# sajadn/Exemplar-VAE

Hardware: AMD Instinct MI355X
Metric: training images/sec (higher is better)
Workload: dtype f32

## Files before the change

### exemplar-vae_amd/csrc/evae_prior.hip

```cpp
#include <algorithm>
#include <type_traits>
#include "evae_tile.h"
#include "evae_prior_gemm.h"

namespace evae {

constexpr long long kMaskAll = EVAE_PRIOR_MASK_ALL;

__device__ __forceinline__ float setup_sigma(float* __restrict__ inv_sigma, float* __restrict__ red,
                                             const float* __restrict__ log_var, int zdim, int zpad) {
  float part = 0.f;
  for (int k = threadIdx.x; k < zpad; k += NT) {
    float lv = k < zdim ? log_var[k] : 0.f;
    inv_sigma[k] = k < zdim ? expf(-0.5f * lv) : 0.f;
    if (k < zdim) part += lv + kLog2Pi;
  }
  part = wave_sum(part);
  if ((threadIdx.x & 63) == 0) red[threadIdx.x >> 6] = part;
  __syncthreads();
  float tot = red[0] + red[1] + red[2] + red[3];
  return -0.5f * tot;
}

template <int KC>
// ... 1719 lines not shown
  return check_launch("prior_bwd_finish_kernel");
}

extern "C" int evae_prior_train_step(const float* z, int B, const float* centres, int C, int zdim, const float* log_var,
                                     const int64_t* z_idx, const int64_t* c_idx, float c_total, const float* beta_dev,
                                     float beta_host, float* logp, float* token, float* cRE, float* cKL, float* neg_cKL,
                                     float* dz, float* dcentres, float* dlogvar, void* state, void* ws, size_t ws_bytes,
                                     int phase, evae_stream_t stream_) {
  return prior_train_step_core(z, B, centres, C, zdim, log_var, z_idx, c_idx, c_total, beta_dev, beta_host, logp, token, cRE, cKL, neg_cKL,
                               dz, dcentres, dlogvar, state, ws, ws_bytes, phase, stream_, nullptr, nullptr, nullptr, 0, nullptr);
}

extern "C" int evae_prior_train_step_rows(const float* z, int B, const float* centres, int n_rows, const int64_t* rows_inv,
                                          const int64_t* rows_rep, const float* rows_mult, int C, int zdim, const float* log_var,
                                          const int64_t* z_idx, const int64_t* c_idx, float c_total, const float* beta_dev,
                                          float beta_host, float* logp, float* token, float* cRE, float* cKL, float* neg_cKL,
                                          float* dz, float* dcentres, float* dc_draws, float* dlogvar, void* state, void* ws,
                                          size_t ws_bytes, evae_stream_t stream_) {
  EVAE_REQUIRE(rows_inv && rows_rep && rows_mult && dc_draws && n_rows >= 1, "prior_train_step_rows: null row tables");
  EVAE_REQUIRE((((uintptr_t)dc_draws | (uintptr_t)dcentres) & 15) == 0, "prior_train_step_rows: gradient buffers must be 16-byte aligned");
  return prior_train_step_core(z, B, centres, C, zdim, log_var, z_idx, c_idx, c_total, beta_dev, beta_host, logp, token, cRE, cKL, neg_cKL,
                               dz, dcentres, dlogvar, state, ws, ws_bytes, 0, stream_, rows_inv, rows_rep, rows_mult, n_rows, dc_draws);
}
```

### exemplar-vae_amd/evae/_lib.py

```python
import ctypes as C
import os

_HERE = os.path.dirname(os.path.abspath(__file__))
LIB_PATH = os.environ.get("EVAE_LIB_PATH") or os.path.join(os.path.dirname(_HERE), "csrc", "libevae_hip.so")

_p = C.c_void_p
_i = C.c_int
_f = C.c_float
_d = C.c_double
_z = C.c_size_t
_l = C.c_int64
_u = C.c_uint
_q = C.c_uint64


class ConvDesc(C.Structure):
    _fields_ = [(n, C.c_int) for n in ("N", "C", "H", "W", "Co", "KH", "KW", "stride", "pad")]


class WtJob(C.Structure):
    _fields_ = [("w1", C.c_void_p), ("w2", C.c_void_p), ("dst", C.c_void_p), ("N", C.c_int), ("K", C.c_int), ("ldt", C.c_int)]


class CtlJob(C.Structure):
# ... 20 lines not shown
class AdamTensor(C.Structure):
    _fields_ = [("param", _p), ("grad", _p), ("exp_avg", _p), ("exp_avg_sq", _p), ("numel", _l)]


SIGNATURES = {
    "evae_version": (_i, []),
    "evae_last_error": (C.c_char_p, []),
    "evae_ctl_upload": (_i, [_p, _p, _p, _z, _p, _p, _p, _p]),
    "evae_host_dedup": (_i, [_p, _i, C.c_int64, _i, _p, _p, _p, _p]),
    "evae_prior_set_norm_limit": (_i, [_f]),
    "evae_prior_lse_fwd_workspace_bytes": (_z, [_i, _i, _i]),
    "evae_prior_lse_fwd": (_i, [_p, _i, _p, _i, _i, _p, _p, _p, _p, _p, _p, _p, _p, _z, _p]),
    "evae_prior_merge": (_i, [_p, _p, _p, _i, _i, _f, _p, _p, _p]),
    "evae_prior_lse_fwd_splits": (_i, [_p, _i, _p, _i, _i, _p, _p, _p, _p, _z, C.POINTER(C.c_int), C.POINTER(C.c_int), _p]),
    "evae_prior_elbo_fwd": (_i, [_p, _p, _p, _i, _i, _i, _f, _p, _p, _p, _f, _p, _p, _p, _p, _p, _p]),
    "evae_prior_elbo_fwd_coef": (_i, [_p, _p, _p, _i, _i, _i, _f, _p, _p, _p, _f, _p, _p, _p, _p, _p, _p, _p, _p, _p]),
    "evae_prior_merge_coef": (_i, [_p, _p, _p, _i, _i, _i, _f, _p, _f, _p, _p, _p, _p, _p, _p]),
    "evae_elbo_assemble": (_i, [_p, _p, _p, _p, _f, _i, _p, _p, _p, _p]),
    "evae_prior_train_applies": (_i, [_i, _i, _i]),
    "evae_prior_train_gave_up": (_i, [_p, _p]),
    "evae_prior_train_workspace_bytes": (_z, [_i, _i, _i]),
    "evae_prior_train_step": (_i, [_p, _i, _p, _i, _i, _p, _p, _p, _f, _p, _f, _p, _p, _p, _p, _p, _p, _p, _p, _p, _p, _z, _i, _p]),
    "evae_prior_train_step_rows": (_i, [_p, _i, _p, _i, _p, _p, _p, _i, _i, _p, _p, _p, _f, _p, _f, _p, _p, _p, _p, _p, _p, _p, _p, _p, _p, _p, _z, _p]),
    "evae_prior_lse_bwd_workspace_bytes": (_z, [_i, _i, _i]),
    "evae_prior_lse_bwd": (_i, [_p, _i, _p, _i, _i, _p, _p, _p, _p, _p, _p, _p, _p, _p, _z, _p]),
    "evae_prior_lse_bwd_phased": (_i, [_p, _i, _p, _i, _i, _p, _p, _p, _p, _p, _p, _p, _p, _p, _z, _i, _p]),
    "evae_mixture_lse_fwd_workspace_bytes": (_z, [_i, _i, _i]),
    "evae_mixture_lse_fwd": (_i, [_p, _i, _p, _p, _i, _i, _f, _p, _p, _p, _p, _z, _p]),
    "evae_mixture_lse_bwd_workspace_bytes": (_z, [_i, _i, _i]),
    "evae_mixture_lse_bwd": (_i, [_p, _i, _p, _p, _i, _i, _p, _p, _p, _p, _p, _p, _z, _p]),
    "evae_pseudo_inputs_fwd": (_i, [_p, _i, _i, _p, _p]),
    "evae_pseudo_inputs_bwd": (_i, [_p, _p, _i, _i, _p, _p]),
    "evae_pairdist_topk_workspace_bytes": (_z, [_i, _i, _i, _i]),
    "evae_pairdist_topk": (_i, [_p, _i, _p, _i, _i, _i, _u, _l, _p, _p, _p, _z, _p]),
    "evae_pairwise_distance": (_i, [_p, _i, _p, _i, _i, _p, _p]),
    "evae_topk_merge": (_i, [_p, _p, _i, _i, _i, _p, _p, _p]),
    "evae_select_exemplars": (_i, [_p, _i, _p, _i, _p, _p, _p, _p]),
    "evae_dense_fwd_workspace_bytes": (_z, [_i, _i, _i, _i]),
    "evae_gated_dense_fwd": (_i, [_p, _p, _i, _i, _i, _p, _p, _p, _p, _i, _p, _p, _p, _p, _z, _p]),
    "evae_linear_fwd": (_i, [_p, _p, _i, _i, _i, _p, _p, _i, _i, _f, _f, _p, _p, _p, _z, _p]),
    "evae_heads_reparam_fwd_workspace_bytes": (_z, [_i, _i, _i]),
    "evae_heads_reparam_fwd": (_i, [_p, _i, _i, _i, _p, _p, _p, _p, _i, _f, _f, _p, _p, _p, _p, _p, _p, _p, _z, _p]),
    "evae_heads_reparam_fwd_bcast_applies": (_i, [_i, _i, _i, _i]),
    "evae_heads_reparam_fwd_bcast": (_i, [_p, _i, _i, _i, _p, _p, _p, _p, _i, _f, _f, _p, _p, _p, _p, _p, _p, _p, _p, _i, _p]),
    "evae_heads_std_applies": (_i, [_i, _i, _i, _i]),
    "evae_heads_reparam_std_fwd": (_i, [_p, _i, _i, _i, _p, _p, _p, _p, _i, _f, _f, _p, _p, _p, _p, _p, _p, _p, _p]),
# ... 12 lines not shown
    "evae_dense_bwd_weight_phased": (_i, [_p, _i, _i, _i, _p, _p, _i, _i, _p, _p, _i, _p, _z, _i, _p]),
    "evae_dense_u8_supported": (_i, [_i, C.c_longlong]),
    "evae_dense_u8_block_rows": (_i, [_i, _i, _i]),
    "evae_dense_u8_prepared_bytes": (_z, [_i, _i]),
    "evae_dense_u8_prepare": (_i, [_p, _p, _i, _i, _p, _z, _p]),
    "evae_gated_dense_fwd_u8": (_i, [_p, _p, _i, _i, C.c_longlong, _f, _p, _p, _p, _i, _p, _p, _p]),
    "evae_dense_bwd_weight_u8_workspace_bytes": (_z, [_i, _i, _i]),
    "evae_dense_bwd_weight_u8": (_i, [_p, _i, _i, C.c_longlong, _p, _p, _i, C.c_longlong, _f, _p, _p, _p, _z, _p]),
    "evae_dense_bwd_weight_u8_phased": (_i, [_p, _i, _i, C.c_longlong, _p, _p, _i, C.c_longlong, _f, _p, _p, _p, _z, _i, _p]),
    "evae_dense_bwd_weight_u8_images": (_i, [_i, _i, _i, C.POINTER(C.c_size_t), C.POINTER(C.c_int)]),
    "evae_broadcast_scalar": (_i, [_p, _p, _i, _p]),
    "evae_sum_small": (_i, [_p, _i, _p, _p]),
    "evae_thin_configure": (_i, [_i]),
    "evae_p6_nks": (_i, [_i]),
    "evae_p6_nks_rows": (_i, [_i]),
    "evae_p6_image_bytes": (_z, [_i, _i]),
    "evae_gemm_p6_applies": (_i, [_i, _i, _i]),
    "evae_p6_pack_rows": (_i, [_p, _p, _i, _i, C.c_longlong, _i, _p, _z, _p]),
    "evae_p6_pack_cols": (_i, [_p, _p, _i, _i, C.c_longlong, _i, _i, _p, _z, _p]),
    "evae_p6_fill_row": (_i, [_p, _i, _i, _f, _i, _i, _p]),
    "evae_gated_dense_fwd_timg": (_i, [_p, _p, _i, _i, _i, _p, _p, _p, _p, _i, _p, _p, _p, _p, _i, _i, _i, _p, _z, _p]),
    "evae_gated_dense_fwd_u8_timg": (_i, [_p, _p, _i, _i, C.c_longlong, _f, _p, _p, _p, _i, _p, _p, _p, _i, _i, _i, _p]),
    "evae_dense_bwd_data_timg": (_i, [_p, _p, _p, _p, _i, _i, _i, _i, _p, _p, _p, _p, _i, _p, _p, _i, _i, _i, _p, _z, _p]),
    "evae_gated_dense_fwd_p6t": (_i, [_p, _i, _i, _i, _p, _p, _p, _i, _p, _p, _p]),
    "evae_dense_bwd_data_p6t": (_i, [_p, _i, _i, _i, _p, _i, _p, _p, _p, _p, _i, _p, _i, _i, _p]),
    "evae_dense_bwd_weight_p6_workspace_bytes": (_z, [_i, _i, _i]),
    "evae_dense_bwd_weight_p6": (_i, [_p, _p, _i, _i, _i, _p, _p, _p, _z, _p]),
    "evae_dense_bwd_data_img": (_i, [_p, _p, _p, _p, _i, _i, _i, _i, _p, _p, _p, _i, _i, _p, _p, _z, _p]),
    "evae_dense_bwd_weight_group": (_i, [_p, _i, _p]),
    "evae_dense_bwd_weight_finish_group": (_i, [_p, _i, _p]),
    "evae_gated_dense_bwd_input": (_i, [_p, _p, _p, _i, _i, _p, _p, _i, _p]),
    "evae_gated_dense_bwd_input_ld": (_i, [_p, _i, _p, _p, _i, _i, _p, _p, _i, _p]),
    "evae_gather_rows": (_i, [_p, _p, _p, _i, _i, _p, _p]),
    "evae_gated_dense_bwd": (_i, [_p, _i, _p, _p, _i, _i, _p, _p, _i, _p, _i, _p, _i, _p, _z, _p]),
    "evae_act_bwd": (_i, [_p, _p, _z, _i, _f, _f, _p, _p]),
    "evae_conv2d_workspace_bytes": (_z, [_p, _i, _i]),
    "evae_conv2d_fwd": (_i, [_p, _p, _p, _p, _p, _p, _i, _f, _f, _p, _p, _p, _p, _z, _p]),
    "evae_conv2d_bwd_data": (_i, [_p, _p, _p, _p, _p, _p, _p, _z, _p]),
    "evae_conv2d_bwd_weight": (_i, [_p, _p, _p, _p, _p, _p, _p, _z, _p]),
    "evae_conv2d_cl_supported": (_i, [_p, _i, _i]),
    "evae_conv2d_cl_dy_stride": (_i, [_i]),
    "evae_conv2d_cl_workspace_bytes": (_z, [_p, _i, _i]),
    "evae_conv2d_cl_fwd": (_i, [_p, _p, _p, _p, _p, _p, _i, _f, _f, _p, _p, _p, _p, _z, _p]),
    "evae_conv2d_cl_bwd_data": (_i, [_p, _p, _p, _p, _p, _p, _z, _p]),
    "evae_conv2d_cl_bwd_weight": (_i, [_p, _p, _p, _i, _p, _p, _p, _z, _p]),
    "evae_gemm_x6_configure": (_i, [_i, _i]),
# ... 123 lines not shown
```

### exemplar-vae_amd/evae/fused_vae.py

```python
import ctypes as C
import os

import torch
import torch.distributed as dist

from . import _lib, handoff, ops, shard

ACT_NONE, ACT_SIGMOID, ACT_HARDTANH = ops.ACT_NONE, ops.ACT_SIGMOID, ops.ACT_HARDTANH

_STAGE_GEN = {}
_XT_GEN = {}
_ZEROED = {}
def node_merge(Cl, B):
    e = os.environ.get("EVAE_NODE_MERGE")
    if e is not None:
        return int(e)
    return 15 if Cl + B <= 8192 else 11


ONE_STREAM = [os.environ.get("EVAE_ONE_STREAM", "0") == "1"]
_APPROX_ROWS = {}

SCHED = int(os.environ.get("EVAE_SCHED", "0"))
FINISH_GROUP_HEAD = os.environ.get("EVAE_FINISH_GROUP_HEAD", "0") == "1"
FINISH_GROUP = os.environ.get("EVAE_FINISH_GROUP", "0") == "1"
HEADW_EARLY = int(os.environ.get("EVAE_HEADW_EARLY", "0"))
ELBO_SPLIT = os.environ.get("EVAE_ELBO_SPLIT", "0") != "0"
PRIOR_TRAIN = os.environ.get("EVAE_PRIOR_TRAIN", "1") != "0"
GROUP_LEAVES = os.environ.get("EVAE_GROUP_LEAVES", "1") != "0"
IMG_DGRAD = os.environ.get("EVAE_IMG_DGRAD", "1") != "0" or bool(SCHED & 4)
THIN_ROWS = 1024
P6 = os.environ.get("EVAE_P6", "1") != "0"
_P6_READY = {}
_ONES = {}

PARAM_ORDER = [
    "prior_log_variance",
    "p_x_mean.linear.weight", "p_x_mean.linear.bias",
    "q_z_layers.0.h.weight", "q_z_layers.0.h.bias", "q_z_layers.0.g.weight", "q_z_layers.0.g.bias",
    "q_z_layers.1.h.weight", "q_z_layers.1.h.bias", "q_z_layers.1.g.weight", "q_z_layers.1.g.bias",
    "q_z_mean.weight", "q_z_mean.bias",
    "q_z_logvar.linear.weight", "q_z_logvar.linear.bias",
    "p_x_layers.0.h.weight", "p_x_layers.0.h.bias", "p_x_layers.0.g.weight", "p_x_layers.0.g.bias",
    "p_x_layers.1.h.weight", "p_x_layers.1.h.bias", "p_x_layers.1.g.weight", "p_x_layers.1.g.bias",
]




def _vp(v):
    if v is None:
        return None
    return C.c_void_p(v if isinstance(v, int) else v.data_ptr())


# ... 268 lines not shown
                           lambda: _lib.check(lib.evae_gated_dense_fwd_p6t(_vp(t_h1), nks_m, Cl, H, _vp(w2_img), _vp(b2h), _vp(b2g), H,
                                                                           _vp(A2), _vp(s2), k.st), "gated_fwd_p6t"),
                           executed=6 * fl2, pipe="bf16-mfma")
            else:
                k.gated_fwd(A1, None, Cl, H, H, w2h, b2h, w2g, b2g, H, A2, None, s2)
            k.linear_fwd(A2, Cl, H, H, wm, bm, Z, ACT_NONE, 0.0, 0.0, mean_all, None)
        if approx:
            approx_cache.index_copy_(0, sel_rows, centres)
        main.wait_event(z_ready)
        centres_p = centres
        if dd is not None and not prior_train:
            centres_p = torch.empty((Cp, Z), **f32)
            _lib.check(lib.evae_gather_rows(_vp(centres), _vp(dd[1]), None, Cp, Z, _vp(centres_p), k.st), "gather_rows(centres)")
        zi = None if no_mask else ops._i64(x_idx)
        ci = None if no_mask else (ci_sel if approx else ops._i64(dd[0] if dd is not None else ex_idx))
        logp = torch.empty(B, **f32); lse = torch.empty((2, B), **f32)
        z_all, zi_all = z, zi
        prior_done = None
        if prior_train:
            dmean_all = torch.empty((Mp, Z), **f32)
            packed = torch.empty(B * Z + Z, **f32)
            ev_pre = torch.cuda.Event(); ev_pre.record()
            keep_alive = None
            if dd is not None:
                dc_x = torch.empty((Cp, Z), **f32)
                keep_alive = [dc_x]
                if os.environ.get("EVAE_PRIOR_ROWS", "1") != "0":
                    ops.prior_train_step_rows(z, centres, (dd[1], dd[2], dd[3]), lv_row, zi, ci, float(c_total),
                                              beta_dev if beta_dev is not None else beta_host,
                                              out=(logp, lse, None, packed[:B * Z].view(B, Z), dmean_all[:Cl], packed[B * Z:]), dc_draws=dc_x,
                                              stream=k.st)
                else:
                    centres_x = torch.empty((Cp, Z), **f32)
                    keep_alive.append(centres_x)
                    _lib.check(lib.evae_gather_rows(_vp(centres), _vp(dd[1]), None, Cp, Z, _vp(centres_x), k.st), "gather_rows(centres)")
                    ops.prior_train_step(z, centres_x, lv_row, zi, ci, float(c_total), beta_dev if beta_dev is not None else beta_host,
                                         out=(logp, lse, None, packed[:B * Z].view(B, Z), dc_x, packed[B * Z:]), stream=k.st)
                    _lib.check(lib.evae_gather_rows(_vp(dc_x), _vp(dd[2]), _vp(dd[3]), Cl, Z, _vp(dmean_all), k.st), "gather_rows(dcentres)")
            else:
                ops.prior_train_step(z, centres, lv_row, zi, ci, float(c_total), beta_dev if beta_dev is not None else beta_host,
                                     out=(logp, lse, None, packed[:B * Z].view(B, Z), dmean_all[:Cl], packed[B * Z:]), stream=k.st)
            prior_done = (dmean_all, packed, ev_pre, keep_alive)
        if sharded == 2:
            z_all = shard._all_gather_flat(z).reshape(-1, Z)
            zi_all = None if zi is None else shard._all_gather_flat(zi.contiguous()).reshape(-1)
            m, s, n, _ = ops.prior_lse_fwd(z_all, centres_p, lv_row, zi_all, ci)
            m, s, n = shard.gather_partials(m, s, n)
            r0 = dist.get_rank() * B
            m, s, n = (t[:, r0:r0 + B].contiguous() for t in (m, s, n))
        elif sharded:
            m, s, n, _ = ops.prior_lse_fwd(z, centres_p, lv_row, zi, ci)
            m, s, n = shard.gather_partials(m, s, n)
        if sharded:
            R, ldp = m.shape[0], m.shape[1]
            pm, ps, pn = m, s, n
        elif prior_train:
            pass
        else:
            nb = lib.evae_prior_lse_fwd_workspace_bytes(B, Cp, Z)
            w = k.ws("prior_fwd", nb)
            ns, prow = C.c_int(0), C.c_int(0)
            _lib.check(lib.evae_prior_lse_fwd_splits(_vp(z), B, _vp(centres_p), Cp, Z, _vp(lv_row), _vp(zi), _vp(ci), _vp(w),
                                                     w.numel(), C.byref(ns), C.byref(prow), k.st), "prior_lse_fwd_splits")
            R, ldp = ns.value, B
            pm = w.data_ptr(); ps = pm + 4 * prow.value * B; pn = ps + 4 * prow.value * B
# ... 130 lines not shown
                fl_ = 2.0 * M * 2 * H * H
                ex_, pipe_ = ops.gemm_pipe(M, H, False, fl_)
                ops.probed("dense_bwd_data M=%d N=%d+%d K=%d (gate-backward epilogue -> bf16 tile images)" % (M, H, H, H), fl_,
                           lambda: _lib.check(lib.evae_dense_bwd_data_img(
                               _vp(dq2.data_ptr() + ob * 2 * H), _vp(w2h), _vp(dq2.data_ptr() + ob * 2 * H + 4 * H), _vp(w2g), M, H,
                               2 * H, H, _vp(A1.data_ptr() + ob * H), _vp(s1.data_ptr() + ob * H), _vp(img_ptr), nslab_img.value,
                               m_base, _vp(wT), _vp(wd), wd.numel(), kk.st), "bwd_data_img"), executed=ex_, pipe=pipe_)
        else:
            def l2_dgrad(kk, M, ob, m_base):
                kk.bwd_data(dq2.data_ptr() + ob * 2 * H, w2h, dq2.data_ptr() + ob * 2 * H + 4 * H, w2g, M, H, 2 * H, H,
                            A1.data_ptr() + ob * H, s1.data_ptr() + ob * H, dq1.data_ptr() + ob * 2 * H,
                            dq1.data_ptr() + ob * 2 * H + 4 * H, 2 * H,
                            wT=None if (ctx.wt is None or kk is not k) else ctx.wt[1])
        dpx_done = ctx.dpx is not None and ctx.coef is not None and cRE is ctx.coef[0]
        dpx = ctx.dpx if dpx_done else torch.empty((B, D), **f32)
        dp2 = torch.empty((B, 2 * H), **f32)
        dp1 = torch.empty((B, 2 * H), **f32)
        dz = torch.empty((B, Z), **f32)
        dlvp = torch.empty((B, Z), **f32)
        centres = mean_all[:Cl]
        z_mean = mean_all[Cl:]
        off = 4 * Cl
        prior_finish = None
        dd_, centres_p = ctx.dd if ctx.dd is not None else (None, centres)
        Cp = centres_p.shape[0]
        dc_out = torch.empty((Cp, Z), **f32) if dd_ is not None else dmean_all

        def dc_fold():
            if dd_ is not None:
                _lib.check(lib.evae_gather_rows(_vp(dc_out), _vp(dd_[2]), _vp(dd_[3]), Cl, Z, _vp(dmean_all), k.st), "gather_rows(dcentres)")
        if prior_done:
            side.wait_event(ctx.prior_done[2])
        else:
            side.wait_stream(main)
        if sharded == 2:
            z_all, zi_all = ctx.dp
            RB = z_all.shape[0]
            lg = shard._all_gather_flat(torch.cat((lse.reshape(2, B), gp.reshape(1, B))))
            lse_all = torch.stack((lg[:, 0].reshape(-1), lg[:, 1].reshape(-1))).contiguous()
            gp_all = lg[:, 2].reshape(-1).contiguous()
            dz_all = torch.empty((RB, Z), **f32); dlv = torch.empty(Z, **f32)
            nb = lib.evae_prior_lse_bwd_workspace_bytes(RB, Cp, Z)
            w = k.ws("prior_bwd", nb)
            _lib.check(lib.evae_prior_lse_bwd(_vp(z_all), RB, _vp(centres_p), Cp, Z, _vp(lv_row), _vp(zi_all), _vp(ci), _vp(lse_all),
                                              _vp(gp_all), _vp(dz_all), _vp(dc_out), _vp(dlv), _vp(w), w.numel(), k.st),
                       "prior_bwd")
            dc_fold()
            dist.all_reduce(dz_all, op=dist.ReduceOp.SUM)
            r0 = dist.get_rank() * B
            dzp = dz_all[r0:r0 + B]
        elif prior_done:
            packed = ctx.prior_done[1]
            dzp = packed[:B * Z].view(B, Z); dlv = packed[B * Z:]
        else:
            assert ctx.prior_done is None, "fused vae step: the captured form's backward was called with another upstream gradient"
            packed = torch.empty(B * Z + Z, **f32)
            dzp = packed[:B * Z].view(B, Z); dlv = packed[B * Z:]
            nb = lib.evae_prior_lse_bwd_workspace_bytes(B, Cp, Z)
            w = k.ws("prior_bwd", nb)
            pb_args = (_vp(z), B, _vp(centres_p), Cp, Z, _vp(lv_row), _vp(zi), _vp(ci), _vp(lse), _vp(gp), _vp(dzp),
                       _vp(dc_out), _vp(dlv), _vp(w), w.numel())
            if sharded == 1 or dd_ is not None or not (SCHED & 1):
                _lib.check(lib.evae_prior_lse_bwd(*pb_args, k.st), "prior_bwd")
                dc_fold()
                if sharded == 1:
                    dist.all_reduce(packed, op=dist.ReduceOp.SUM)
                    if Cl > 0:
                        dmean_all[:Cl].mul_(float(dist.get_world_size()))
            else:
                _lib.check(lib.evae_prior_lse_bwd_phased(*pb_args, 1, k.st), "prior_bwd(1)")
                prior_finish = lambda: _lib.check(lib.evae_prior_lse_bwd_phased(*pb_args, 2, kd.st), "prior_bwd(2)")
        dz_ready = torch.cuda.Event(); dz_ready.record()
        if Cl > 0:
            if p6:
                nbh = lib.evae_dense_bwd_data_workspace_bytes(Cl, Z, H, 1)
                wh_ = k.ws("dgrad", nbh)
                flh = 2.0 * Cl * Z * H
                exh, pih = ops.gemm_pipe(Cl, H, False, flh)
                ops.probed("dense_bwd_data M=%d N=%d K=%d (gate-backward epilogue -> pre-split image)" % (Cl, Z, H), flh,
                           hbm_bytes=4.0 * Cl * (Z + 2 * H) + 6.0 * Cl * 2 * H, fn=
                           lambda: _lib.check(lib.evae_dense_bwd_data_timg(_vp(dmean_all), _vp(wm), None, None, Cl, Z, Z, H, _vp(A2), _vp(s2),
                                                                           None, None, 2 * H, _vp(None if ctx.wt is None else ctx.wt[0]),
                                                                           _vp(t_dq2), nks_m, 0, 0, _vp(wh_), wh_.numel(), k.st),
                                              "bwd_data_timg"))
            else:
                k.bwd_data(dmean_all, wm, None, None, Cl, Z, Z, H, A2, s2, dq2, dq2.data_ptr() + 4 * H, 2 * H,
                           wT=None if ctx.wt is None else ctx.wt[0])
            l2_dgrad(k, Cl, 0, 0)
        batch_rows_done = torch.cuda.Event()
        g_plv = gslot("plv", 1)
        g_wp = gslot("wp", D, H); g_bp = gslot("bp", D)
        g_d2 = gslot("d2", 2 * H, H); g_e2 = gslot("e2", 2 * H)
        g_d1 = gslot("d1", 2 * H, Z); g_e1 = gslot("e1", 2 * H)
        g_wl = gslot("wl", Z, H); g_bl = gslot("bl", Z)
        g_wm = gslot("wm", Z, H); g_bm = gslot("bm", Z)
        fin_group = FINISH_GROUP and data_ext.dtype == torch.uint8 and not (SCHED & 10) and Mp > 128 and not p6
        headw_early = bool(HEADW_EARLY and not fin_group and Cl > 0)
# ... 157 lines not shown
```

### exemplar-vae_amd/evae/ops.py

```python
import ctypes as C
import os

import torch

from . import _lib, handoff

ACT_NONE, ACT_SIGMOID, ACT_HARDTANH = 0, 1, 2
TOPK_SQRT = 1

_ws = {}
_ws_retired = []
PROBE = None


def probed(name, flops, fn, executed=None, pipe="fp32-mfma", min_flops=2e9, hbm_bytes=None):
    if PROBE is None or (flops < PROBE.get("min_flops", min_flops) if hbm_bytes is None else hbm_bytes < 16e6):
        return fn()
    if hbm_bytes is not None:
        flops, executed, pipe = hbm_bytes, hbm_bytes, "hbm"
    e0 = torch.cuda.Event(enable_timing=True); e1 = torch.cuda.Event(enable_timing=True)
    e0.record()
    r = fn()
    e1.record()
    PROBE["records"].append((name, e0, e1, float(flops), float(executed if executed is not None else flops), pipe))
# ... 159 lines not shown
    key = (device.index if device.index is not None else torch.cuda.current_device(), tag)
    st = _PT_STATE.get(key)
    if st is None:
        st = _PT_STATE[key] = torch.zeros(64, dtype=torch.int32, device=device)
    return st


def prior_train_check():
    lib = _lib.load()
    for key, st in list(_PT_STATE.items()):
        n = lib.evae_prior_train_gave_up(_p(st), torch.cuda.current_stream(st.device).cuda_stream)
        if n < 0:
            _lib.check(n, "evae_prior_train_gave_up")
        if n > 0:
            raise RuntimeError("evae: %d block(s) of the one-launch exemplar prior gave up waiting for the rest of their grid (device "
                               "%s): gradients of at least one step are wrong.  The grid was not co-resident -- set "
                               "EVAE_PRIOR_TRAIN=0 to use the three-launch prior on this device" % (n, key[0]))


def prior_train_applies(B, Cn, zd):
    return bool(_lib.load().evae_prior_train_applies(int(B), int(Cn), int(zd)))


def prior_train_step_rows(z, centres, rows, log_var, z_idx, c_idx, c_total, beta, out, dc_draws, stream=None):
    lib = _lib.load()
    inv, rep, mult = rows
    B, zd = z.shape
    Cn = inv.numel()
    logp, token, coef, dz, dc, dlv = out
    beta_dev = beta if torch.is_tensor(beta) else None
    ws = _workspace("prior_train", lib.evae_prior_train_workspace_bytes(B, Cn, zd), z.device)
    st = prior_train_state(z.device)
    c3 = coef if coef is not None else (None, None, None)
    _lib.check(lib.evae_prior_train_step_rows(_p(z), B, _p(centres), centres.shape[0], _p(inv), _p(rep), _p(mult), Cn, zd, _p(log_var),
                                              _p(_i64(z_idx)), _p(_i64(c_idx)), float(c_total), _p(beta_dev),
                                              0.0 if beta_dev is not None else float(beta), _p(logp), _p(token), _p(c3[0]), _p(c3[1]),
                                              _p(c3[2]), _p(dz), _p(dc), _p(dc_draws), _p(dlv), _p(st), _p(ws), ws.numel(),
                                              _stream() if stream is None else stream), "evae_prior_train_step_rows")
    return out


def prior_train_step(z, centres, log_var, z_idx, c_idx, c_total, beta, want_coef=True, out=None, phase=0, stream=None):
    lib = _lib.load()
    _need_cuda(z, centres, log_var, z_idx, c_idx)
    z, centres, log_var = _f32(z), _f32(centres), _f32(log_var).reshape(-1)
    B, zd = z.shape
    Cn = centres.shape[0]
    z_idx, c_idx = _i64(z_idx), _i64(c_idx)
    if z_idx is None or c_idx is None:
        z_idx = c_idx = None
    dev = z.device
    if out is None:
        f = dict(device=dev, dtype=torch.float32)
        coef = (torch.empty(B, **f), torch.empty(B, **f), torch.empty(B, **f)) if want_coef else None
        out = (torch.empty(B, **f), torch.empty((2, B), **f), coef, torch.empty((B, zd), **f), torch.empty((Cn, zd), **f), torch.empty(zd, **f))
    logp, token, coef, dz, dc, dlv = out
    beta_dev = beta if torch.is_tensor(beta) else None
    ws = _workspace("prior_train", lib.evae_prior_train_workspace_bytes(B, Cn, zd), dev)
    st = prior_train_state(dev)
    c3 = coef if coef is not None else (None, None, None)
    _lib.check(lib.evae_prior_train_step(_p(z), B, _p(centres), Cn, zd, _p(log_var), _p(z_idx), _p(c_idx), float(c_total), _p(beta_dev),
# ... 2059 lines not shown
```

### include/evae_hip.h

```cpp
#ifndef EVAE_HIP_H
#define EVAE_HIP_H

#include <stddef.h>
#include <stdint.h>

#ifdef __cplusplus
extern "C" {
#endif

#define EVAE_OK 0
#define EVAE_EINVAL (-1)
#define EVAE_EWORKSPACE (-2)
#define EVAE_ELAUNCH (-3)

#define EVAE_ABI_VERSION 1

typedef void* evae_stream_t;

int evae_version(void);
const char* evae_last_error(void);
int evae_ctl_upload(void* d_stage, const void* h_pinned, void* d_ctl, size_t bytes, evae_stream_t up, evae_stream_t step,
                    void* ev_used, void* ev_up);

int evae_host_dedup(const int64_t* draws, int n_draws, int64_t n_rows, int cap, int64_t* rows, int64_t* inv, int64_t* rep, float* mult);
// ... 22 lines not shown
                             const float* RE, const float* logq, const float* beta_dev, float beta_host, float* logp, float* lse,
                             float* loss, float* KL, float* means, float* cRE, float* cKL, float* neg_cKL, evae_stream_t stream);

int evae_prior_merge_coef(const float* pmax, const float* psum, const float* pnmask, int R, int ldp, int B, float c_total,
                          const float* beta_dev, float beta_host, float* logp , float* lse ,
                          float* cRE, float* cKL, float* neg_cKL, evae_stream_t stream);
int evae_elbo_assemble(const float* logp, const float* RE, const float* logq, const float* beta_dev, float beta_host, int B,
                       float* loss , float* KL , float* means , evae_stream_t stream);

int evae_prior_train_applies(int B, int C, int zdim);
int evae_prior_train_gave_up(void* state, evae_stream_t stream);
size_t evae_prior_train_workspace_bytes(int B, int C, int zdim);
int evae_prior_train_step(const float* z, int B, const float* centres, int C, int zdim, const float* log_var,
                          const int64_t* z_idx, const int64_t* c_idx, float c_total, const float* beta_dev, float beta_host,
                          float* logp , float* token , float* cRE, float* cKL, float* neg_cKL,
                          float* dz , float* dcentres , float* dlogvar , void* state,
                          void* ws, size_t ws_bytes, int phase, evae_stream_t stream);
int evae_prior_train_step_rows(const float* z, int B, const float* centres, int n_rows, const int64_t* rows_inv, const int64_t* rows_rep,
                               const float* rows_mult, int C, int zdim, const float* log_var, const int64_t* z_idx,
                               const int64_t* c_idx, float c_total, const float* beta_dev, float beta_host, float* logp, float* token,
                               float* cRE, float* cKL, float* neg_cKL, float* dz, float* dcentres ,
                               float* dc_draws , float* dlogvar, void* state, void* ws, size_t ws_bytes,
                               evae_stream_t stream);

size_t evae_prior_lse_bwd_workspace_bytes(int B, int C, int zdim);
int evae_prior_lse_bwd(const float* z, int B, const float* centres, int C, int zdim,
                       const float* log_var, const int64_t* z_idx, const int64_t* c_idx,
                       const float* lse , const float* grad_out ,
                       float* dz , float* dcentres ,
                       float* dlogvar ,
                       void* ws, size_t ws_bytes, evae_stream_t stream);
int evae_prior_lse_bwd_phased(const float* z, int B, const float* centres, int C, int zdim, const float* log_var,
                              const int64_t* z_idx, const int64_t* c_idx, const float* lse, const float* grad_out,
                              float* dz, float* dcentres, float* dlogvar, void* ws, size_t ws_bytes, int phase,
                              evae_stream_t stream);

size_t evae_mixture_lse_fwd_workspace_bytes(int B, int C, int zdim);
int evae_mixture_lse_fwd(const float* z , int B, const float* means ,
                         const float* log_var , int C, int zdim, float n_components,
                         float* out_logp , float* out_lse ,
                         float* out_prob , void* ws, size_t ws_bytes, evae_stream_t stream);
size_t evae_mixture_lse_bwd_workspace_bytes(int B, int C, int zdim);
int evae_mixture_lse_bwd(const float* z, int B, const float* means, const float* log_var, int C, int zdim,
                         const float* lse , const float* grad_out ,
                         float* dz , float* dmeans ,
                         float* dlog_var , void* ws, size_t ws_bytes, evae_stream_t stream);
// ... 222 lines not shown
                  evae_stream_t stream);
int evae_step_stats_add(const float* loss, const float* re, const float* kl, float* step3, float* totals3,
                        evae_stream_t stream);
int evae_thin_configure(int max_rows);
int evae_p6_nks(int K);
int evae_p6_nks_rows(int M);
size_t evae_p6_image_bytes(int rows, int nks);
int evae_gemm_p6_applies(int M, int N, int gated);
int evae_p6_pack_rows(const float* x, const float* x2 , int R, int K, long long ld, int gated, void* img,
                      size_t img_bytes, evae_stream_t stream);
int evae_p6_pack_cols(const float* x, const float* x2 , int Kd, int R, long long ld, int ones_row ,
                      int nks, void* img, size_t img_bytes, evae_stream_t stream);
int evae_p6_fill_row(void* img, int nks, int row, float value, int k_begin, int k_end, evae_stream_t stream);
int evae_gated_dense_fwd_timg(const float* x, const int64_t* rows, int M, int K, int ldx, const float* wh, const float* bh,
                              const float* wg, const float* bg, int N, float* out, float* save_h, float* save_s,
                              void* timg, int t_nks, int t_row0, int t_kbase, void* ws, size_t ws_bytes, evae_stream_t stream);
int evae_gated_dense_fwd_u8_timg(const unsigned char* x, const int64_t* rows, int M, int K, long long ldx, float x_scale,
                                 const void* prepared, const float* bh, const float* bg, int N, float* out, float* save_s,
                                 void* timg, int t_nks, int t_row0, int t_kbase, evae_stream_t stream);
int evae_dense_bwd_data_timg(const float* dy1, const float* w1, const float* dy2, const float* w2, int M, int N, int ldy, int K,
                             const float* out_prev, const float* s_prev, float* dx_or_dh, float* dg, int ldo,
                             const float* wT , void* timg, int t_nks, int t_row0, int t_kbase, void* ws,
                             size_t ws_bytes, evae_stream_t stream);
int evae_gated_dense_fwd_p6t(const void* xT_img, int x_nks, int M, int K, const void* w_img, const float* bh, const float* bg,
                             int N, float* out , float* save_s , evae_stream_t stream);
int evae_dense_bwd_data_p6t(const void* dyT_img, int dy_nks, int M, int N, const void* wT_img, int K, const float* out_prev,
                            const float* s_prev, float* dh, float* dg, int ldo, void* u8_img, int u8_nslab, int u8_mbase,
                            evae_stream_t stream);
size_t evae_dense_bwd_weight_p6_workspace_bytes(int nks, int N, int K);
int evae_dense_bwd_weight_p6(const void* dyT_img, const void* xT_img, int nks, int N, int K, float* dw ,
                             float* db , void* ws, size_t ws_bytes,
                             evae_stream_t stream);
int evae_broadcast_scalar(const float* src, float* dst, int n, evae_stream_t stream);
int evae_sum_small(const float* x, int n, float* out, evae_stream_t stream);
int evae_batch_prologue(const float* data, int64_t ldd, const int64_t* idx, int B, int D, int binarize,
                        const int64_t* seed_ctr , float* x_out, int64_t ldx,
                        float* eps_out , int zdim, evae_stream_t stream);
int evae_batch_prologue_u8(const unsigned char* data, int64_t ldd, const int64_t* idx, int B, int D, int binarize,
                           const int64_t* seed_ctr, float x_div, float* x_out, int64_t ldx, unsigned char* stage, int64_t lds,
                           float* eps_out, int zdim, evae_stream_t stream);
typedef struct { const float* w1; const float* w2; float* dst; int N, K, ldt; } evae_wt_job_t;
int evae_batch_prologue_u8_prepare(const unsigned char* data, int64_t ldd, const int64_t* idx, int B, int D, int binarize,
                                   const int64_t* seed_ctr, float x_div, float* x_out, int64_t ldx, unsigned char* stage,
                                   int64_t lds, float* eps_out, int zdim, const float* wh, const float* wg, int N, int K,
                                   void* prepared, size_t prepared_bytes, const evae_wt_job_t* jobs, int njobs,
                                   evae_stream_t stream);
// ... 45 lines not shown
```

Baseline: 200,800.

## Add streaming narrow-heads backward-data kernel reading prior row tables directly

Adds a dedicated MFMA kernel for the heads backward-data product with a small latent dimension (Z up to 64). It computes the gate backward and writes straight into the pre-split image. It can read the exemplar gradient from the prior's per-draw tables (dc_draws scaled by rows_mult) instead of a materialised dcentres buffer. A phased prior step is also added so the prior's final scatter can be deferred off the critical path. This replaces the general dense dgrad path for the narrow heads, cutting its workspace traffic and a launch, but adds a new specialised kernel and a split prior schedule.

```diff
diff --git a/exemplar-vae_amd/csrc/evae_narrow_heads.hip b/exemplar-vae_amd/csrc/evae_narrow_heads.hip
--- /dev/null
+++ b/exemplar-vae_amd/csrc/evae_narrow_heads.hip
@@ -0,0 +1,133 @@
+
+#include "evae_common.h"
+#include "evae_p6_image.h"
+
+namespace evae {
+
+typedef float f32x16 __attribute__((ext_vector_type(16)));
+
+constexpr int HB_TILES = 8;
+
+template <int Z8>
+__global__ __launch_bounds__(64 * HB_TILES) void heads_bwd_data_timg_kernel(const float* __restrict__ dy, int ldy,
+                                                                           const float* __restrict__ dc_draws,
+                                                                           const int64_t* __restrict__ rows_rep,
+                                                                           const float* __restrict__ rows_mult,
+                                                                           const float* __restrict__ w, int M, int Z, int H,
+                                                                           const float* __restrict__ a, const float* __restrict__ s,
+                                                                           float* __restrict__ dh, float* __restrict__ dg, int ldo,
+                                                                           P6Sink sink, int tiles_per_block) {
+  constexpr int ZP = 8 * Z8, NS = 4 * Z8;
+  __shared__ float sdy[ZP * 33];
+  const int tid = threadIdx.x, wv = tid >> 6, l = tid & 63, l31 = l & 31, lh = l >> 5;
+  const int m0 = blockIdx.x * 32;
+  const int h = (blockIdx.y * tiles_per_block + wv) * 32 + l31;
+  const bool hok = h < H;
+  float bf[NS];
+#pragma unroll
+  for (int st = 0; st < NS; ++st) {
+    const int k = 2 * st + lh;
+    bf[st] = (hok && k < Z) ? w[(size_t)k * H + h] : 0.f;
+  }
+  float av[16], sv[16];
+#pragma unroll
+  for (int r = 0; r < 16; ++r) {
+    const int m = m0 + (r & 3) + 8 * (r >> 2) + 4 * lh;
+    const bool ok = hok && m < M;
+    const size_t oe = (size_t)(ok ? m : 0) * H + (ok ? h : 0);
+    const float a_ = a[oe], s_ = s[oe];
+    av[r] = ok ? a_ : 0.f;
+    sv[r] = ok ? s_ : 0.f;
+  }
+  const int Z4 = Z >> 2;
+  for (int i = tid; i < 32 * (ZP / 4); i += blockDim.x) {
+    const int r = i / (ZP / 4), c = i - r * (ZP / 4);
+    const int m = m0 + r;
+    float4 v = make_float4(0.f, 0.f, 0.f, 0.f);
+    if (m < M && c < Z4) {
+      if (rows_rep) {
+        const float mu = rows_mult[m];
+        const float4 d = *reinterpret_cast<const float4*>(dc_draws + (size_t)rows_rep[m] * Z + 4 * c);
+        v = make_float4(mu * d.x, mu * d.y, mu * d.z, mu * d.w);
+      } else {
+        v = *reinterpret_cast<const float4*>(dy + (size_t)m * ldy + 4 * c);
+      }
+    }
+    sdy[(4 * c + 0) * 33 + r] = v.x; sdy[(4 * c + 1) * 33 + r] = v.y;
+    sdy[(4 * c + 2) * 33 + r] = v.z; sdy[(4 * c + 3) * 33 + r] = v.w;
+  }
+  __syncthreads();
+  f32x16 acc;
+#pragma unroll
+  for (int r = 0; r < 16; ++r) acc[r] = 0.f;
+#pragma unroll
+  for (int st = 0; st < NS; ++st)
+    acc = __builtin_amdgcn_mfma_f32_32x32x2f32(sdy[(2 * st + lh) * 33 + l31], bf[st], acc, 0, 0, 0);
+  float dhv[16], dgv[16];
+#pragma unroll
+  for (int r = 0; r < 16; ++r) {
+    const float v = acc[r], s_ = sv[r];
+    dhv[r] = v * s_;
+    dgv[r] = v * av[r] * (1.0f - s_);
+  }
+  if (dh) {
+#pragma unroll
+    for (int r = 0; r < 16; ++r) {
+      const int m = m0 + (r & 3) + 8 * (r >> 2) + 4 * lh;
+      if (hok && m < M) {
+        const size_t o = (size_t)m * ldo + h;
+        dh[o] = dhv[r];
+        dg[o] = dgv[r];
+      }
+    }
+  }
+  const int k0 = sink.kbase + m0;
+  p6_emit_tile(sink, sink.row0 + h, hok, k0, dhv, lh);
+  p6_emit_tile(sink, sink.row0 + H + h, hok, k0, dgv, lh);
+}
+
+}
+
+using namespace evae;
+
+extern "C" int evae_heads_bwd_data_timg_applies(int M, int Z, int H) {
+  return (M >= 1 && Z >= 4 && Z <= 64 && Z % 4 == 0 && H >= 1 && H <= 32 * HB_TILES * 65535) ? 1 : 0;
+}
+
+extern "C" int evae_heads_bwd_data_timg(const float* dy, const float* w, int M, int Z, int ldy, int H, const float* out_prev,
+                                        const float* s_prev, float* dh, float* dg, int ldo, void* timg, int t_nks, int t_row0,
+                                        int t_kbase, const float* dc_draws, const int64_t* rows_rep, const float* rows_mult,
+                                        evae_stream_t stream_) {
+  hipStream_t stream = (hipStream_t)stream_;
+  EVAE_REQUIRE(M >= 0, "heads_bwd_data_timg: bad row count %d", M);
+  if (M == 0) return EVAE_OK;
+  EVAE_REQUIRE(evae_heads_bwd_data_timg_applies(M, Z, H), "heads_bwd_data_timg: M=%d Z=%d H=%d is outside the streaming form "
+               "(Z <= 64 and a multiple of 4)", M, Z, H);
+  const bool tables = dc_draws || rows_rep || rows_mult;
+  EVAE_REQUIRE(!tables || (dc_draws && rows_rep && rows_mult), "heads_bwd_data_timg: all three row tables or none");
+  EVAE_REQUIRE(tables || (dy && ldy >= Z && ldy % 4 == 0), "heads_bwd_data_timg: dy missing or its row stride %d not a multiple of 4", ldy);
+  EVAE_REQUIRE(w && out_prev && s_prev, "heads_bwd_data_timg: null pointer");
+  EVAE_REQUIRE((dh == nullptr) == (dg == nullptr) && (!dh || ldo >= H), "heads_bwd_data_timg: dh and dg together, ldo >= H");
+  EVAE_REQUIRE(((((uintptr_t)(tables ? dc_draws : dy)) | ((uintptr_t)timg)) & 15) == 0,
+               "heads_bwd_data_timg: dy / dc_draws and the image must be 16-byte aligned");
+  EVAE_REQUIRE(timg && t_nks > 0 && t_row0 >= 0 && t_kbase >= 0 && (t_kbase % 8) == 0 && (t_kbase + M + 15) / 16 <= t_nks,
+               "heads_bwd_data_timg: bad image placement (k-steps %d, first k %d, rows %d)", t_nks, t_kbase, M);
+  const P6Sink sink = {(unsigned char*)timg, t_nks, t_row0, t_kbase, t_kbase + M};
+  const int tiles = cdiv(H, 32), gy = cdiv(tiles, HB_TILES), tpb = cdiv(tiles, gy);
+  const dim3 grid(cdiv(M, 32), gy);
+#define EVAE_HB(Z8_) heads_bwd_data_timg_kernel<Z8_><<<grid, 64 * tpb, 0, stream>>>(tables ? nullptr : dy, ldy, dc_draws, rows_rep, \
+                                                                                     rows_mult, w, M, Z, H, out_prev, s_prev, dh, dg, \
+                                                                                     ldo, sink, tpb)
+  switch (cdiv(Z, 8)) {
+    case 1: EVAE_HB(1); break;
+    case 2: EVAE_HB(2); break;
+    case 3: EVAE_HB(3); break;
+    case 4: EVAE_HB(4); break;
+    case 5: EVAE_HB(5); break;
+    case 6: EVAE_HB(6); break;
+    case 7: EVAE_HB(7); break;
+    default: EVAE_HB(8); break;
+  }
+#undef EVAE_HB
+  return check_launch("heads_bwd_data_timg_kernel");
+}
diff --git a/exemplar-vae_amd/csrc/evae_prior.hip b/exemplar-vae_amd/csrc/evae_prior.hip
--- a/exemplar-vae_amd/csrc/evae_prior.hip
+++ b/exemplar-vae_amd/csrc/evae_prior.hip
@@ -1765,3 +1765,16 @@
   return prior_train_step_core(z, B, centres, C, zdim, log_var, z_idx, c_idx, c_total, beta_dev, beta_host, logp, token, cRE, cKL, neg_cKL,
                                dz, dcentres, dlogvar, state, ws, ws_bytes, 0, stream_, rows_inv, rows_rep, rows_mult, n_rows, dc_draws);
 }
+
+extern "C" int evae_prior_train_step_rows_phased(const float* z, int B, const float* centres, int n_rows, const int64_t* rows_inv,
+                                                 const int64_t* rows_rep, const float* rows_mult, int C, int zdim,
+                                                 const float* log_var, const int64_t* z_idx, const int64_t* c_idx, float c_total,
+                                                 const float* beta_dev, float beta_host, float* logp, float* token, float* cRE,
+                                                 float* cKL, float* neg_cKL, float* dz, float* dcentres, float* dc_draws,
+                                                 float* dlogvar, void* state, void* ws, size_t ws_bytes, int phase,
+                                                 evae_stream_t stream_) {
+  EVAE_REQUIRE(rows_inv && rows_rep && rows_mult && dc_draws && n_rows >= 1, "prior_train_step_rows: null row tables");
+  EVAE_REQUIRE((((uintptr_t)dc_draws | (uintptr_t)dcentres) & 15) == 0, "prior_train_step_rows: gradient buffers must be 16-byte aligned");
+  return prior_train_step_core(z, B, centres, C, zdim, log_var, z_idx, c_idx, c_total, beta_dev, beta_host, logp, token, cRE, cKL, neg_cKL,
+                               dz, dcentres, dlogvar, state, ws, ws_bytes, phase, stream_, rows_inv, rows_rep, rows_mult, n_rows, dc_draws);
+}
diff --git a/exemplar-vae_amd/evae/_lib.py b/exemplar-vae_amd/evae/_lib.py
--- a/exemplar-vae_amd/evae/_lib.py
+++ b/exemplar-vae_amd/evae/_lib.py
@@ -66,6 +66,7 @@
     "evae_prior_train_workspace_bytes": (_z, [_i, _i, _i]),
     "evae_prior_train_step": (_i, [_p, _i, _p, _i, _i, _p, _p, _p, _f, _p, _f, _p, _p, _p, _p, _p, _p, _p, _p, _p, _p, _z, _i, _p]),
     "evae_prior_train_step_rows": (_i, [_p, _i, _p, _i, _p, _p, _p, _i, _i, _p, _p, _p, _f, _p, _f, _p, _p, _p, _p, _p, _p, _p, _p, _p, _p, _p, _z, _p]),
+    "evae_prior_train_step_rows_phased": (_i, [_p, _i, _p, _i, _p, _p, _p, _i, _i, _p, _p, _p, _f, _p, _f, _p, _p, _p, _p, _p, _p, _p, _p, _p, _p, _p, _z, _i, _p]),
     "evae_prior_lse_bwd_workspace_bytes": (_z, [_i, _i, _i]),
     "evae_prior_lse_bwd": (_i, [_p, _i, _p, _i, _i, _p, _p, _p, _p, _p, _p, _p, _p, _p, _z, _p]),
     "evae_prior_lse_bwd_phased": (_i, [_p, _i, _p, _i, _i, _p, _p, _p, _p, _p, _p, _p, _p, _p, _z, _i, _p]),
@@ -124,6 +125,8 @@
     "evae_gated_dense_fwd_timg": (_i, [_p, _p, _i, _i, _i, _p, _p, _p, _p, _i, _p, _p, _p, _p, _i, _i, _i, _p, _z, _p]),
     "evae_gated_dense_fwd_u8_timg": (_i, [_p, _p, _i, _i, C.c_longlong, _f, _p, _p, _p, _i, _p, _p, _p, _i, _i, _i, _p]),
     "evae_dense_bwd_data_timg": (_i, [_p, _p, _p, _p, _i, _i, _i, _i, _p, _p, _p, _p, _i, _p, _p, _i, _i, _i, _p, _z, _p]),
+    "evae_heads_bwd_data_timg_applies": (_i, [_i, _i, _i]),
+    "evae_heads_bwd_data_timg": (_i, [_p, _p, _i, _i, _i, _i, _p, _p, _p, _p, _i, _p, _i, _i, _i, _p, _p, _p, _p]),
     "evae_gated_dense_fwd_p6t": (_i, [_p, _i, _i, _i, _p, _p, _p, _i, _p, _p, _p]),
     "evae_dense_bwd_data_p6t": (_i, [_p, _i, _i, _i, _p, _i, _p, _p, _p, _p, _i, _p, _i, _i, _p]),
     "evae_dense_bwd_weight_p6_workspace_bytes": (_z, [_i, _i, _i]),
diff --git a/exemplar-vae_amd/evae/fused_vae.py b/exemplar-vae_amd/evae/fused_vae.py
--- a/exemplar-vae_amd/evae/fused_vae.py
+++ b/exemplar-vae_amd/evae/fused_vae.py
@@ -31,6 +31,7 @@
 IMG_DGRAD = os.environ.get("EVAE_IMG_DGRAD", "1") != "0" or bool(SCHED & 4)
 THIN_ROWS = 1024
 P6 = os.environ.get("EVAE_P6", "1") != "0"
+NARROW_HEADS = [int(os.environ.get("EVAE_NARROW_HEADS", "6"))]
 _P6_READY = {}
 _ONES = {}
 
@@ -345,14 +346,19 @@
             packed = torch.empty(B * Z + Z, **f32)
             ev_pre = torch.cuda.Event(); ev_pre.record()
             keep_alive = None
+            heads_rows = None
             if dd is not None:
                 dc_x = torch.empty((Cp, Z), **f32)
                 keep_alive = [dc_x]
                 if os.environ.get("EVAE_PRIOR_ROWS", "1") != "0":
-                    ops.prior_train_step_rows(z, centres, (dd[1], dd[2], dd[3]), lv_row, zi, ci, float(c_total),
-                                              beta_dev if beta_dev is not None else beta_host,
-                                              out=(logp, lse, None, packed[:B * Z].view(B, Z), dmean_all[:Cl], packed[B * Z:]), dc_draws=dc_x,
-                                              stream=k.st)
+                    heads_tables = bool(p6 and (NARROW_HEADS[0] & 2) and lib.evae_heads_bwd_data_timg_applies(Cl, Z, H))
+                    finish_late = bool(heads_tables and (NARROW_HEADS[0] & 4))
+                    pt_args = (z, centres, (dd[1], dd[2], dd[3]), lv_row, zi, ci, float(c_total),
+                               beta_dev if beta_dev is not None else beta_host)
+                    pt_out = (logp, lse, None, packed[:B * Z].view(B, Z), dmean_all[:Cl], packed[B * Z:])
+                    ops.prior_train_step_rows(*pt_args, out=pt_out, dc_draws=dc_x, stream=k.st, phase=1 if finish_late else 0)
+                    if heads_tables:
+                        heads_rows = (dc_x, dd[2], dd[3], (pt_args, pt_out) if finish_late else None)
                 else:
                     centres_x = torch.empty((Cp, Z), **f32)
                     keep_alive.append(centres_x)
@@ -363,7 +369,7 @@
             else:
                 ops.prior_train_step(z, centres, lv_row, zi, ci, float(c_total), beta_dev if beta_dev is not None else beta_host,
                                      out=(logp, lse, None, packed[:B * Z].view(B, Z), dmean_all[:Cl], packed[B * Z:]), stream=k.st)
-            prior_done = (dmean_all, packed, ev_pre, keep_alive)
+            prior_done = (dmean_all, packed, ev_pre, keep_alive, heads_rows)
         if sharded == 2:
             z_all = shard._all_gather_flat(z).reshape(-1, Z)
             zi_all = None if zi is None else shard._all_gather_flat(zi.contiguous()).reshape(-1)
@@ -540,6 +546,7 @@
         z_mean = mean_all[Cl:]
         off = 4 * Cl
         prior_finish = None
+        heads_rows = None
         dd_, centres_p = ctx.dd if ctx.dd is not None else (None, centres)
         Cp = centres_p.shape[0]
         dc_out = torch.empty((Cp, Z), **f32) if dd_ is not None else dmean_all
@@ -570,6 +577,10 @@
         elif prior_done:
             packed = ctx.prior_done[1]
             dzp = packed[:B * Z].view(B, Z); dlv = packed[B * Z:]
+            heads_rows = ctx.prior_done[4]
+            if heads_rows is not None and heads_rows[3] is not None:
+                pt_args, pt_out = heads_rows[3]
+                prior_finish = lambda: ops.prior_train_step_rows(*pt_args, out=pt_out, dc_draws=heads_rows[0], stream=kd.st, phase=2)
         else:
             assert ctx.prior_done is None, "fused vae step: the captured form's backward was called with another upstream gradient"
             packed = torch.empty(B * Z + Z, **f32)
@@ -590,7 +601,14 @@
                 prior_finish = lambda: _lib.check(lib.evae_prior_lse_bwd_phased(*pb_args, 2, kd.st), "prior_bwd(2)")
         dz_ready = torch.cuda.Event(); dz_ready.record()
         if Cl > 0:
-            if p6:
+            if p6 and (NARROW_HEADS[0] & 2) and lib.evae_heads_bwd_data_timg_applies(Cl, Z, H):
+                dc_, rep_, mult_ = heads_rows[:3] if heads_rows is not None else (None, None, None)
+                ops.probed("dense_bwd_data M=%d N=%d K=%d (heads, streaming: gate-backward -> pre-split image)" % (Cl, Z, H),
+                           2.0 * Cl * Z * H, hbm_bytes=4.0 * Cl * (Z + 2 * H) + 6.0 * Cl * 2 * H, fn=
+                           lambda: _lib.check(lib.evae_heads_bwd_data_timg(_vp(None if dc_ is not None else dmean_all), _vp(wm), Cl, Z, Z, H,
+                                                                           _vp(A2), _vp(s2), None, None, 2 * H, _vp(t_dq2), nks_m, 0, 0,
+                                                                           _vp(dc_), _vp(rep_), _vp(mult_), k.st), "heads_bwd_data_timg"))
+            elif p6:
                 nbh = lib.evae_dense_bwd_data_workspace_bytes(Cl, Z, H, 1)
                 wh_ = k.ws("dgrad", nbh)
                 flh = 2.0 * Cl * Z * H
diff --git a/exemplar-vae_amd/evae/ops.py b/exemplar-vae_amd/evae/ops.py
--- a/exemplar-vae_amd/evae/ops.py
+++ b/exemplar-vae_amd/evae/ops.py
@@ -205,7 +205,7 @@
     return bool(_lib.load().evae_prior_train_applies(int(B), int(Cn), int(zd)))
 
 
-def prior_train_step_rows(z, centres, rows, log_var, z_idx, c_idx, c_total, beta, out, dc_draws, stream=None):
+def prior_train_step_rows(z, centres, rows, log_var, z_idx, c_idx, c_total, beta, out, dc_draws, stream=None, phase=0):
     lib = _lib.load()
     inv, rep, mult = rows
     B, zd = z.shape
@@ -215,11 +215,14 @@
     ws = _workspace("prior_train", lib.evae_prior_train_workspace_bytes(B, Cn, zd), z.device)
     st = prior_train_state(z.device)
     c3 = coef if coef is not None else (None, None, None)
-    _lib.check(lib.evae_prior_train_step_rows(_p(z), B, _p(centres), centres.shape[0], _p(inv), _p(rep), _p(mult), Cn, zd, _p(log_var),
-                                              _p(_i64(z_idx)), _p(_i64(c_idx)), float(c_total), _p(beta_dev),
-                                              0.0 if beta_dev is not None else float(beta), _p(logp), _p(token), _p(c3[0]), _p(c3[1]),
-                                              _p(c3[2]), _p(dz), _p(dc), _p(dc_draws), _p(dlv), _p(st), _p(ws), ws.numel(),
-                                              _stream() if stream is None else stream), "evae_prior_train_step_rows")
+    args = (_p(z), B, _p(centres), centres.shape[0], _p(inv), _p(rep), _p(mult), Cn, zd, _p(log_var), _p(_i64(z_idx)), _p(_i64(c_idx)),
+            float(c_total), _p(beta_dev), 0.0 if beta_dev is not None else float(beta), _p(logp), _p(token), _p(c3[0]), _p(c3[1]),
+            _p(c3[2]), _p(dz), _p(dc), _p(dc_draws), _p(dlv), _p(st), _p(ws), ws.numel())
+    st_ = _stream() if stream is None else stream
+    if phase:
+        _lib.check(lib.evae_prior_train_step_rows_phased(*args, int(phase), st_), "evae_prior_train_step_rows_phased")
+    else:
+        _lib.check(lib.evae_prior_train_step_rows(*args, st_), "evae_prior_train_step_rows")
     return out
 
 
diff --git a/include/evae_hip.h b/include/evae_hip.h
--- a/include/evae_hip.h
+++ b/include/evae_hip.h
@@ -68,6 +68,12 @@
                                float* cRE, float* cKL, float* neg_cKL, float* dz, float* dcentres ,
                                float* dc_draws , float* dlogvar, void* state, void* ws, size_t ws_bytes,
                                evae_stream_t stream);
+int evae_prior_train_step_rows_phased(const float* z, int B, const float* centres, int n_rows, const int64_t* rows_inv,
+                                      const int64_t* rows_rep, const float* rows_mult, int C, int zdim, const float* log_var,
+                                      const int64_t* z_idx, const int64_t* c_idx, float c_total, const float* beta_dev,
+                                      float beta_host, float* logp, float* token, float* cRE, float* cKL, float* neg_cKL, float* dz,
+                                      float* dcentres, float* dc_draws, float* dlogvar, void* state, void* ws, size_t ws_bytes,
+                                      int phase, evae_stream_t stream);
 
 size_t evae_prior_lse_bwd_workspace_bytes(int B, int C, int zdim);
 int evae_prior_lse_bwd(const float* z, int B, const float* centres, int C, int zdim,
@@ -336,6 +342,11 @@
                              const float* out_prev, const float* s_prev, float* dx_or_dh, float* dg, int ldo,
                              const float* wT , void* timg, int t_nks, int t_row0, int t_kbase, void* ws,
                              size_t ws_bytes, evae_stream_t stream);
+int evae_heads_bwd_data_timg_applies(int M, int Z, int H);
+int evae_heads_bwd_data_timg(const float* dy, const float* w, int M, int Z, int ldy, int H, const float* out_prev,
+                             const float* s_prev, float* dh, float* dg, int ldo, void* timg, int t_nks, int t_row0, int t_kbase,
+                             const float* dc_draws , const int64_t* rows_rep ,
+                             const float* rows_mult , evae_stream_t stream);
 int evae_gated_dense_fwd_p6t(const void* xT_img, int x_nks, int M, int K, const void* w_img, const float* bh, const float* bg,
                              int N, float* out , float* save_s , evae_stream_t stream);
 int evae_dense_bwd_data_p6t(const void* dyT_img, int dy_nks, int M, int N, const void* wT_img, int K, const float* out_prev,
```

After: 204,500, median of 6. +1.8%, better.
